# nrsyed/pytorch-yolov3

Hardware: AMD Instinct MI355X
Metric: frames/sec (608x608) (higher is better)
Workload: dtype bf16

## Files before the change

pytorch-yolov3_amd/csrc/conv_fused.hip:

```cpp
#include "common.h"
#include <type_traits>

namespace {

constexpr int kTO = 16;
constexpr int kSR = 2 * kTO + 1;
constexpr int kIR = kSR + 2;
constexpr int kInPitch = 144;
constexpr int kStemPitch = 80;
constexpr int kW1Pitch = 608;
constexpr int kNStem = kSR * kSR;
constexpr int kNFrag = (kNStem + 15) / 16;
constexpr int kThreads = 512;
constexpr int kInBytes = kIR * kInPitch * 2;
constexpr int kPatchElems = kIR * kIR * 3;
constexpr int kPre = (kPatchElems + kThreads - 1) / kThreads;
constexpr int kLds = 2 * kInBytes + kNStem * kStemPitch + 64 * kW1Pitch + 512;

template <typename T>
struct FusedArgs {
  const unsigned char *in;
  int H, W, batch;
  const T *w0;
  const float *sc0, *bi0;
  uint32_t flags0;
  const T *w1;
  int k_ld1;
  const float *sc1, *bi1;
  uint32_t flags1;
  T *out;
  int out_ld, Ho, Wo;
  int tiles_x, tiles_y, n_tiles;
  int dbg;
};

template <typename T>
__device__ __forceinline__ u32x2 bn_leaky_pack4(const f32x4 &a, const f32x4 &sc, const f32x4 &bi) {
  const f32x2 lo = f32x2{a[0], a[1]} * f32x2{sc[0], sc[1]} + f32x2{bi[0], bi[1]};
  const f32x2 hi = f32x2{a[2], a[3]} * f32x2{sc[2], sc[3]} + f32x2{bi[2], bi[3]};
  const f32x2 tl = lo * Y3_LEAKY_SLOPE, th = hi * Y3_LEAKY_SLOPE;
  return y3_pack4<T>(y3_vmax(lo[0], tl[0]), y3_vmax(lo[1], tl[1]), y3_vmax(hi[0], th[0]), y3_vmax(hi[1], th[1]));
}

template <typename T>
__global__ __launch_bounds__(kThreads) void conv_stem_s2_fused_kernel(FusedArgs<T> p) {
  typedef typename H16<T>::v8 V8;
  extern __shared__ __attribute__((aligned(16))) char smem[];
  T *in_tile = reinterpret_cast<T *>(smem);
  char *stem = smem + 2 * kInBytes;
  char *w1s = stem + kNStem * kStemPitch;
  T *lut = reinterpret_cast<T *>(w1s + 64 * kW1Pitch);

  const int tid = threadIdx.x, lane = tid & 63;
  const int wave = __builtin_amdgcn_readfirstlane(tid >> 6);
  const int fr = lane & 15, fq = lane >> 4;

  for (int i = tid; i < 64 * 36; i += kThreads) {
    const int co = i / 36, ch = i - co * 36;
    *reinterpret_cast<u32x4 *>(w1s + co * kW1Pitch + ch * 16) =
        *reinterpret_cast<const u32x4 *>(reinterpret_cast<const char *>(p.w1) + ((long long)co * p.k_ld1) * 2 + ch * 16);
  }
  V8 w0a[2], w0b[2];
#pragma unroll
  for (int st = 0; st < 2; ++st)
#pragma unroll
    for (int j = 0; j < 8; ++j) {
      const int k = st * 32 + fq * 8 + j;
      const int ky = k / 12, rem = k - ky * 12, kx = rem >> 2, c = rem & 3;
      const bool live = k < 36 && c < 3;
      const int kold = live ? ky * 9 + kx * 3 + c : 0;
      const T za = p.w0[(0 + fr) * 32 + kold], zb = p.w0[(16 + fr) * 32 + kold];
      w0a[st][j] = live ? za : (T)0.f;
      w0b[st][j] = live ? zb : (T)0.f;
    }
  int off_lo, off_hi;
  {
    const int k0 = fq * 8, k1 = fq * 8 + 4;
    off_lo = (k0 / 12) * kInPitch + (k0 % 12);
    off_hi = (k1 / 12) * kInPitch + (k1 % 12);
  }
  const int off_s1 = 2 * kInPitch + 8;
  const int cq = fq * 4;
  f32x4 sc0[2], bi0[2];
#pragma unroll
  for (int ni = 0; ni < 2; ++ni) {
    sc0[ni] = *reinterpret_cast<const f32x4 *>(p.sc0 + ni * 16 + cq);
    bi0[ni] = *reinterpret_cast<const f32x4 *>(p.bi0 + ni * 16 + cq);
  }

  int pr_row[kPre], pr_col[kPre], pr_dst[kPre];
  uint32_t pr_goff[kPre];
#pragma unroll
  for (int j = 0; j < kPre; ++j) {
    const int i = tid + j * kThreads;
    const int r = i / (kIR * 3), cb = i - r * (kIR * 3);
    pr_row[j] = r;
    pr_col[j] = cb;
    pr_goff[j] = (uint32_t)(r * p.W * 3 + cb);
    pr_dst[j] = r * kInPitch + (cb / 3) * 4 + (cb % 3);
  }
  const bool pr_last_live = tid + (kPre - 1) * kThreads < kPatchElems;
  auto tile_coords = [&](int tile, int &tx, int &ty, int &b) {
    int t = tile;
    tx = t % p.tiles_x;
    t /= p.tiles_x;
    ty = t % p.tiles_y;
    b = t / p.tiles_y;
  };
  auto patch_fetch = [&](int tile, unsigned char (&pre)[kPre]) {
    int tx, ty, b;
    tile_coords(tile, tx, ty, b);
    const int iy0 = 2 * ty * kTO - 2, ixb0 = (2 * tx * kTO - 2) * 3;
    const bool interior = iy0 >= 0 && iy0 + kIR <= p.H && ixb0 >= 0 && ixb0 + kIR * 3 <= p.W * 3;
    if (interior) {
      const unsigned char *base = p.in + ((long long)b * p.H + iy0) * p.W * 3 + ixb0;
#pragma unroll
      for (int j = 0; j < kPre; ++j) pre[j] = (j < kPre - 1 || pr_last_live) ? base[pr_goff[j]] : (unsigned char)0;
    } else {
#pragma unroll
      for (int j = 0; j < kPre; ++j) {
        const int iy = iy0 + pr_row[j], ixb = ixb0 + pr_col[j];
        unsigned char v = 0;
        if ((j < kPre - 1 || pr_last_live) && (unsigned)iy < (unsigned)p.H && ixb >= 0 && ixb < p.W * 3)
          v = p.in[((long long)b * p.H + iy) * p.W * 3 + ixb];
        pre[j] = v;
      }
    }
  };
  auto patch_store = [&](int buf, const unsigned char (&pre)[kPre]) {
    T *dst = in_tile + buf * (kIR * kInPitch);
#pragma unroll
    for (int j = 0; j < kPre; ++j)
      if (j < kPre - 1 || pr_last_live) dst[pr_dst[j]] = lut[pre[j]];
  };

  for (int i = tid; i < 2 * kIR * kInPitch / 2; i += kThreads) reinterpret_cast<uint32_t *>(in_tile)[i] = 0u;
  if (tid < 256) lut[tid] = (T)((float)tid / 255.0f);
  __syncthreads();
  int tile = blockIdx.x;
  int buf = 0;
  if (tile < p.n_tiles) {
    unsigned char pre[kPre];
    patch_fetch(tile, pre);
    patch_store(0, pre);
  }
  for (; tile < p.n_tiles; tile += gridDim.x) {
    int tx, ty, b;
    tile_coords(tile, tx, ty, b);
    const int oy0 = ty * kTO, ox0 = tx * kTO;
    __syncthreads();

    const T *patch = in_tile + buf * (kIR * kInPitch);
    const bool stem_inside = 2 * oy0 - 1 >= 0 && 2 * oy0 - 1 + kSR <= p.H && 2 * ox0 - 1 >= 0 && 2 * ox0 - 1 + kSR <= p.W;
    constexpr int kFG = 3;
    constexpr int kFragIters = (kNFrag + kThreads / 64 - 1) / (kThreads / 64);
    static_assert(kFragIters % kFG == 0, "fragment groups");
#pragma unroll 1
    for (int g = 0; g < ((p.dbg & 1) ? 0 : kFragIters); g += kFG) {
      u32x2 lo[kFG], hi[kFG], s1[kFG];
      int qv[kFG], syv[kFG], sxv[kFG];
#pragma unroll
      for (int j = 0; j < kFG; ++j) {
        const int q = (wave + (g + j) * (kThreads / 64)) * 16 + fr;
        const int qc = q < kNStem ? q : kNStem - 1;
        const int sy = qc / kSR, sx = qc - sy * kSR;
        const T *base = patch + sy * kInPitch + sx * 4;
        lo[j] = *reinterpret_cast<const u32x2 *>(base + off_lo);
        hi[j] = *reinterpret_cast<const u32x2 *>(base + off_hi);
        s1[j] = *reinterpret_cast<const u32x2 *>(base + off_s1);
        qv[j] = q;
        syv[j] = sy;
        sxv[j] = sx;
      }
      f32x4 acc0[kFG], acc1[kFG];
#pragma unroll
      for (int j = 0; j < kFG; ++j) {
        const V8 xf0 = __builtin_bit_cast(V8, u32x4{lo[j][0], lo[j][1], hi[j][0], hi[j][1]});
        acc0[j] = H16<T>::mfma(w0a[0], xf0, f32x4{0.f, 0.f, 0.f, 0.f});
        acc1[j] = H16<T>::mfma(w0b[0], xf0, f32x4{0.f, 0.f, 0.f, 0.f});
      }
#pragma unroll
      for (int j = 0; j < kFG; ++j) {
        const V8 xf1 = __builtin_bit_cast(V8, fq == 0 ? u32x4{s1[j][0], s1[j][1], 0u, 0u} : u32x4{0u, 0u, 0u, 0u});
        acc0[j] = H16<T>::mfma(w0a[1], xf1, acc0[j]);
        acc1[j] = H16<T>::mfma(w0b[1], xf1, acc1[j]);
      }
#pragma unroll
      for (int j = 0; j < kFG; ++j) {
        if (qv[j] < kNStem) {
          bool inside = true;
          if (!stem_inside) {
            const int gy = 2 * oy0 - 1 + syv[j], gx = 2 * ox0 - 1 + sxv[j];
            inside = (unsigned)gy < (unsigned)p.H && (unsigned)gx < (unsigned)p.W;
          }
#pragma unroll
          for (int ni = 0; ni < 2; ++ni) {
            u32x2 o = bn_leaky_pack4<T>(ni ? acc1[j] : acc0[j], sc0[ni], bi0[ni]);
            if (!inside) o = u32x2{0u, 0u};
            *reinterpret_cast<u32x2 *>(stem + qv[j] * kStemPitch + (ni * 16 + cq) * 2) = o;
          }
        }
      }
    }
    const int next_tile = tile + gridDim.x;
    unsigned char pre[kPre];
    if (next_tile < p.n_tiles && !(p.dbg & 8)) patch_fetch(next_tile, pre);
    __syncthreads();

    f32x4 acc[2][4];
#pragma unroll
    for (int mi = 0; mi < 2; ++mi)
#pragma unroll
      for (int nf = 0; nf < 4; ++nf) acc[mi][nf] = f32x4{0.f, 0.f, 0.f, 0.f};
#pragma unroll
    for (int tap = 0; tap < ((p.dbg & 2) ? 0 : 9); ++tap) {
      const int ky = tap / 3, kx = tap - ky * 3;
      u32x4 xf[2], wf[4];
#pragma unroll
      for (int mi = 0; mi < 2; ++mi) {
        const int q = (2 * (2 * wave + mi) + ky) * kSR + 2 * fr + kx;
        xf[mi] = *reinterpret_cast<const u32x4 *>(stem + q * kStemPitch + fq * 16);
      }
#pragma unroll
      for (int nf = 0; nf < 4; ++nf)
        wf[nf] = *reinterpret_cast<const u32x4 *>(w1s + (nf * 16 + fr) * kW1Pitch + tap * 64 + fq * 16);
#pragma unroll
      for (int mi = 0; mi < 2; ++mi)
#pragma unroll
        for (int nf = 0; nf < 4; ++nf)
          acc[mi][nf] = H16<T>::mfma(__builtin_bit_cast(V8, wf[nf]),
                                                                __builtin_bit_cast(V8, xf[mi]), acc[mi][nf]);
    }
    if (next_tile < p.n_tiles) patch_store(buf ^ 1, pre);
    __syncthreads();

#pragma unroll
    for (int nf = 0; nf < 4; ++nf) {
      const f32x4 s1 = *reinterpret_cast<const f32x4 *>(p.sc1 + nf * 16 + cq);
      const f32x4 b1 = *reinterpret_cast<const f32x4 *>(p.bi1 + nf * 16 + cq);
#pragma unroll
      for (int mi = 0; mi < 2; ++mi) {
        const int px = (2 * wave + mi) * kTO + fr;
        const int co = nf * 16 + cq;
        *reinterpret_cast<u32x2 *>(stem + px * 128 + (((co >> 3) ^ (px & 7)) << 4) + (co & 7) * 2) =
            bn_leaky_pack4<T>(acc[mi][nf], s1, b1);
      }
    }
    __syncthreads();
#pragma unroll
    for (int j = 0; j < kTO * kTO * 8 / kThreads; ++j) {
      const int i = tid + j * kThreads;
      const int px = i >> 3, ch = i & 7;
      const int oy = oy0 + (px >> 4), ox = ox0 + (px & 15);
      if (oy < p.Ho && ox < p.Wo && !(p.dbg & 4)) {
        const u32x4 v = *reinterpret_cast<const u32x4 *>(stem + px * 128 + ((ch ^ (px & 7)) << 4));
        *reinterpret_cast<u32x4 *>(p.out + (((long long)b * p.Ho + oy) * p.Wo + ox) * p.out_ld + ch * 8) = v;
      }
    }
    buf ^= 1;
  }
}


constexpr int kPX = 16, kPY = 8;
constexpr int kPSX = 2 * kPX + 1;
constexpr int kPSY = 2 * kPY + 1;
constexpr int kPIX = kPSX + 2, kPIY = kPSY + 2;
constexpr int kPNStem = kPSX * kPSY;
constexpr int kPNFrag = (kPNStem + 15) / 16;
constexpr int kPInBytes = kPIY * kInPitch * 2;
constexpr int kPStemBytes = kPNStem * kStemPitch;
constexpr int kPStage = 8 * 16 * 128;
constexpr int kPLds = 2 * kPInBytes + 2 * kPStemBytes + 64 * kW1Pitch + 512 + kPStage;
static_assert(kPLds <= 160 * 1024, "LDS budget");
static_assert(kPX == 16 && kPY == 8, "one 16-pixel output row per conv wave");

template <typename T, int NC>
__global__ __launch_bounds__(1024) void conv_stem_s2_ws_kernel(FusedArgs<T> p) {
  typedef typename H16<T>::v8 V8;
  constexpr int NS = 16 - NC, NT = 1024;
  constexpr int MR = kPY / NC;
  constexpr int kIters = (kPNFrag + NS - 1) / NS;
  constexpr int kPairs = kPIY * ((kPIX * 3 + 1) / 2);
  constexpr int kPre = (kPairs + 64 * NS - 1) / (64 * NS);
  extern __shared__ __attribute__((aligned(16))) char smem[];
  char *in_tile = smem;
  char *stem0 = smem + 2 * kPInBytes;
  char *w1s = stem0 + 2 * kPStemBytes;
  T *lut = reinterpret_cast<T *>(w1s + 64 * kW1Pitch);
  char *stage = reinterpret_cast<char *>(lut) + 512;

  const int tid = threadIdx.x, lane = tid & 63;
  const int wave = __builtin_amdgcn_readfirstlane(tid >> 6);
  const int fr = lane & 15, fq = lane >> 4;
  const bool is_stem = wave >= NC;

  for (int i = tid; i < 64 * 36; i += NT) {
    const int j = i / 36, ch = i - j * 36;
    const int co = y3_pair_perm(j);
    *reinterpret_cast<u32x4 *>(w1s + j * kW1Pitch + ch * 16) =
        *reinterpret_cast<const u32x4 *>(reinterpret_cast<const char *>(p.w1) + ((long long)co * p.k_ld1) * 2 + ch * 16);
  }
  for (int i = tid; i < 2 * kPInBytes / 4; i += NT) reinterpret_cast<uint32_t *>(in_tile)[i] = 0u;
  if (tid < 256) lut[tid] = (T)((float)tid / 255.0f);
  __syncthreads();
  const int tile0 = blockIdx.x, stride = gridDim.x;
  if (tile0 >= p.n_tiles) return;
  struct TilePos { int tile, tx, ty, b; };
  auto pos_of = [&](int tile) {
    TilePos t;
    t.tile = tile;
    t.tx = tile % p.tiles_x;
    const int r = tile / p.tiles_x;
    t.ty = r % p.tiles_y;
    t.b = r / p.tiles_y;
    return t;
  };
  const TilePos dpos = pos_of(stride);
  auto advance = [&](TilePos &t) {
    t.tile += stride;
    t.tx += dpos.tx;
    int c = t.tx >= p.tiles_x ? 1 : 0;
    t.tx -= c ? p.tiles_x : 0;
    t.ty += dpos.ty + c;
    c = t.ty >= p.tiles_y ? 1 : 0;
    t.ty -= c ? p.tiles_y : 0;
    t.b += dpos.b + c;
  };

  if (is_stem) {
    const int sw = wave - NC, stid = tid - 64 * NC;
    V8 w0a[2], w0b[2];
#pragma unroll
    for (int st = 0; st < 2; ++st)
#pragma unroll
      for (int j = 0; j < 8; ++j) {
        const int k = st * 32 + fq * 8 + j;
        const int ky = k / 12, rem = k - ky * 12, kx = rem >> 2, c = rem & 3;
        const bool live = k < 36 && c < 3;
        const int kold = live ? ky * 9 + kx * 3 + c : 0;
        const T za = p.w0[y3_pair_perm(fr) * 32 + kold], zb = p.w0[y3_pair_perm(16 + fr) * 32 + kold];
        w0a[st][j] = live ? za : (T)0.f;
        w0b[st][j] = live ? zb : (T)0.f;
      }
    int off_lo, off_hi;
    {
      const int k0 = fq * 8, k1 = fq * 8 + 4;
      off_lo = ((k0 / 12) * kInPitch + (k0 % 12)) * 2;
      off_hi = ((k1 / 12) * kInPitch + (k1 % 12)) * 2;
    }
    constexpr int off_s1 = (2 * kInPitch + 8) * 2;
    f32x4 sc0[2], bi0[2];
#pragma unroll
    for (int ni = 0; ni < 2; ++ni) {
      sc0[ni] = *reinterpret_cast<const f32x4 *>(p.sc0 + fq * 8 + ni * 4);
      bi0[ni] = *reinterpret_cast<const f32x4 *>(p.bi0 + fq * 8 + ni * 4);
    }
    int fr_patch[kIters];
    uint32_t fr_live = 0;
#pragma unroll
    for (int j = 0; j < kIters; ++j) {
      const int q = (sw + NS * j) * 16 + fr;
      const int qc = q < kPNStem ? q : kPNStem - 1;
      const int sy = qc / kPSX, sx = qc - sy * kPSX;
      fr_patch[j] = (sy * kInPitch + sx * 4) * 2;
      fr_live |= (q < kPNStem ? 1u : 0u) << j;
    }
    int stem_wr = ((sw * 16 + fr) * kStemPitch) + fq * 16;
    asm volatile("" : "+v"(stem_wr));
    constexpr int kRowPairs = (kPIX * 3 + 1) / 2;
    int pr_dst[kPre];
    uint32_t pr_goff[kPre];
    uint32_t pr_one = 0;
#pragma unroll
    for (int j = 0; j < kPre; ++j) {
      const int i = stid + j * 64 * NS;
      const int r = i / kRowPairs, cb = 2 * (i - r * kRowPairs);
      pr_goff[j] = (uint32_t)(r * p.W * 3 + cb);
      pr_dst[j] = (r * kInPitch + (cb / 3) * 4 + (cb % 3)) * 2 | (cb % 3 == 2 ? 1 : 0);
      pr_one |= (cb + 1 >= kPIX * 3 ? 1u : 0u) << j;
    }
    const bool pr_last_live = stid + (kPre - 1) * 64 * NS < kPairs;
    const bool pairs_aligned = ((p.W * 3) & 1) == 0 && (reinterpret_cast<size_t>(p.in) & 1) == 0;
    auto patch_fetch = [&](const TilePos &t, unsigned short (&pre)[kPre]) {
      const int tx = t.tx, ty = t.ty, b = t.b;
      const int iy0 = 2 * ty * kPY - 2, ixb0 = (2 * tx * kPX - 2) * 3;
      const bool interior = pairs_aligned && iy0 >= 0 && iy0 + kPIY <= p.H && ixb0 >= 0 && ixb0 + 2 * kRowPairs <= p.W * 3;
      if (interior) {
        const unsigned char *base = p.in + ((long long)b * p.H + iy0) * p.W * 3 + ixb0;
#pragma unroll
        for (int j = 0; j < kPre; ++j)
          pre[j] = (j < kPre - 1 || pr_last_live) ? *reinterpret_cast<const unsigned short *>(base + pr_goff[j]) : (unsigned short)0;
      } else {
#pragma unroll
        for (int j = 0; j < kPre; ++j) {
          const int i = stid + j * 64 * NS;
          const int r = i / kRowPairs, cb = 2 * (i - r * kRowPairs);
          const int iy = iy0 + r, ixb = ixb0 + cb;
          unsigned int v = 0;
          if ((j < kPre - 1 || pr_last_live) && (unsigned)iy < (unsigned)p.H) {
            const unsigned char *row = p.in + ((long long)b * p.H + iy) * p.W * 3;
            if (ixb >= 0 && ixb < p.W * 3) v = row[ixb];
            if (ixb + 1 >= 0 && ixb + 1 < p.W * 3 && cb + 1 < kPIX * 3) v |= (unsigned int)row[ixb + 1] << 8;
          }
          pre[j] = (unsigned short)v;
        }
      }
    };
    auto patch_store = [&](int buf, const unsigned short (&pre)[kPre]) {
      char *dst = in_tile + buf * kPInBytes;
#pragma unroll
      for (int j = 0; j < kPre; ++j)
        if (j < kPre - 1 || pr_last_live) {
          char *d = dst + (pr_dst[j] & ~1);
          *reinterpret_cast<T *>(d) = lut[pre[j] & 255];
          if (!((pr_one >> j) & 1u)) *reinterpret_cast<T *>(d + 2 + 2 * (pr_dst[j] & 1)) = lut[pre[j] >> 8];
        }
    };
    auto stem_image = [&](const char *patch, char *img, const TilePos &t) {
      const int oy0 = t.ty * kPY, ox0 = t.tx * kPX;
      const bool all_inside = 2 * oy0 - 1 >= 0 && 2 * oy0 - 1 + kPSY <= p.H && 2 * ox0 - 1 >= 0 && 2 * ox0 - 1 + kPSX <= p.W;
      auto group = [&](auto g0, auto cnt) {
        constexpr int g = decltype(g0)::value, G = decltype(cnt)::value;
        u32x2 lo[G], hi[G], s1[G];
#pragma unroll
        for (int j = 0; j < G; ++j) {
          const char *base = patch + fr_patch[g + j];
          lo[j] = *reinterpret_cast<const u32x2 *>(base + off_lo);
          hi[j] = *reinterpret_cast<const u32x2 *>(base + off_hi);
          s1[j] = *reinterpret_cast<const u32x2 *>(base + off_s1);
        }
        f32x4 a0[G], a1[G];
#pragma unroll
        for (int j = 0; j < G; ++j) {
          const V8 xf0 = __builtin_bit_cast(V8, u32x4{lo[j][0], lo[j][1], hi[j][0], hi[j][1]});
          a0[j] = H16<T>::mfma(w0a[0], xf0, f32x4{0.f, 0.f, 0.f, 0.f});
          a1[j] = H16<T>::mfma(w0b[0], xf0, f32x4{0.f, 0.f, 0.f, 0.f});
        }
#pragma unroll
        for (int j = 0; j < G; ++j) {
          const V8 xf1 = __builtin_bit_cast(V8, u32x4{s1[j][0], s1[j][1], s1[j][0], s1[j][1]});
          a0[j] = H16<T>::mfma(w0a[1], xf1, a0[j]);
          a1[j] = H16<T>::mfma(w0b[1], xf1, a1[j]);
        }
#pragma unroll
        for (int j = 0; j < G; ++j) {
          u32x2 o0 = bn_leaky_pack4<T>(a0[j], sc0[0], bi0[0]);
          u32x2 o1 = bn_leaky_pack4<T>(a1[j], sc0[1], bi0[1]);
          if (!all_inside) {
            const int q = (sw + NS * (g + j)) * 16 + fr;
            const int qc = q < kPNStem ? q : kPNStem - 1;
            const int sy = qc / kPSX, sx = qc - sy * kPSX;
            const int gy = 2 * oy0 - 1 + sy, gx = 2 * ox0 - 1 + sx;
            if (!((unsigned)gy < (unsigned)p.H && (unsigned)gx < (unsigned)p.W)) {
              o0 = u32x2{0u, 0u};
              o1 = u32x2{0u, 0u};
            }
          }
          if ((fr_live >> (g + j)) & 1u) {
            char *dst = img + stem_wr + (g + j) * (NS * 16 * kStemPitch);
            *reinterpret_cast<u32x4 *>(dst) = u32x4{o0[0], o0[1], o1[0], o1[1]};
          }
        }
      };
      using std::integral_constant;
      static_assert(kIters == 5 || kIters == 3, "fragment groups");
      group(integral_constant<int, 0>{}, integral_constant<int, 3>{});
      if constexpr (kIters == 5) group(integral_constant<int, 3>{}, integral_constant<int, 2>{});
    };

    unsigned short pre[4][kPre];
    TilePos fpos = pos_of(tile0);
    TilePos ipos = fpos;
    {
      patch_fetch(fpos, pre[0]);
      patch_store(0, pre[0]);
      advance(fpos);
      if (fpos.tile < p.n_tiles) {
        patch_fetch(fpos, pre[1]);
        patch_store(1, pre[1]);
      }
      advance(fpos);
    }
    __builtin_amdgcn_s_waitcnt(0xC07F);
    __builtin_amdgcn_s_barrier();
#pragma unroll
    for (int k = 0; k < 3; ++k) {
      if (fpos.tile < p.n_tiles) patch_fetch(fpos, pre[k]);
      advance(fpos);
    }
    stem_image(in_tile, stem0, ipos);
    advance(ipos);
    __builtin_amdgcn_s_waitcnt(0xC07F);
    __builtin_amdgcn_s_barrier();
    int par = 0;
    Y3_STAMP_DECL
    auto step = [&](auto setc) {
      constexpr int set = decltype(setc)::value;
      if (fpos.tile < p.n_tiles) patch_fetch(fpos, pre[(set + 3) & 3]);
      advance(fpos);
      Y3_STAMP(0);
      const bool more = ipos.tile < p.n_tiles;
      if (more) stem_image(in_tile + (par ^ 1) * kPInBytes, stem0 + (par ^ 1) * kPStemBytes, ipos);
      advance(ipos);
      __builtin_amdgcn_s_waitcnt(0xC07F);
      Y3_STAMP(1);
      if (ipos.tile < p.n_tiles) patch_store(par, pre[set]);
      __builtin_amdgcn_s_waitcnt(0xC07F);
      Y3_STAMP(2);
      __builtin_amdgcn_s_barrier();
      Y3_STAMP(3);
      par ^= 1;
      return more;
    };
    using std::integral_constant;
    for (;;) {
      if (!step(integral_constant<int, 0>{})) break;
      if (!step(integral_constant<int, 1>{})) break;
      if (!step(integral_constant<int, 2>{})) break;
      if (!step(integral_constant<int, 3>{})) break;
    }
#ifdef Y3_STAMPS
    if (tid == 64 * NC) for (int _i = 0; _i < 4; ++_i) atomicAdd(&g_y3_stamps[_i], _st_acc[_i]);
#endif
    return;
  }

  const int a_rd = ((2 * wave * MR) * kPSX + 2 * fr) * kStemPitch + fq * 16;
  const int b_rd = fr * kW1Pitch + fq * 16;
  char *my_stage = stage + wave * (MR * 16 * 128);
  f32x4 s1v[4], b1v[4];
#pragma unroll
  for (int nf = 0; nf < 4; ++nf) {
    s1v[nf] = *reinterpret_cast<const f32x4 *>(p.sc1 + (nf >> 1) * 32 + fq * 8 + (nf & 1) * 4);
    b1v[nf] = *reinterpret_cast<const f32x4 *>(p.bi1 + (nf >> 1) * 32 + fq * 8 + (nf & 1) * 4);
  }
  __builtin_amdgcn_s_waitcnt(0xC07F);
  __builtin_amdgcn_s_barrier();
  __builtin_amdgcn_s_barrier();
  uint32_t st_off[2];
#pragma unroll
  for (int k = 0; k < 2; ++k) st_off[k] = (uint32_t)((((lane >> 3) + 8 * k) * p.out_ld + (lane & 7) * 8) * 2);
  int par = 0;
  Y3_STAMP_DECL
  for (TilePos pos = pos_of(tile0); pos.tile < p.n_tiles; advance(pos)) {
    const int b = pos.b;
    const int oy0 = pos.ty * kPY, ox0 = pos.tx * kPX;
    const char *img = stem0 + par * kPStemBytes;
    f32x4 acc[MR][4];
#pragma unroll
    for (int mr = 0; mr < MR; ++mr)
#pragma unroll
      for (int nf = 0; nf < 4; ++nf) acc[mr][nf] = f32x4{0.f, 0.f, 0.f, 0.f};
#pragma unroll
    for (int tap = 0; tap < 9; ++tap) {
      const int ky = tap / 3, kx = tap - ky * 3;
      u32x4 xf[MR], wf[4];
#pragma unroll
      for (int mr = 0; mr < MR; ++mr)
        xf[mr] = *reinterpret_cast<const u32x4 *>(img + a_rd + ((2 * mr + ky) * kPSX + kx) * kStemPitch);
#pragma unroll
      for (int nf = 0; nf < 4; ++nf)
        wf[nf] = *reinterpret_cast<const u32x4 *>(w1s + b_rd + nf * 16 * kW1Pitch + tap * 64);
#pragma unroll
      for (int mr = 0; mr < MR; ++mr)
#pragma unroll
        for (int nf = 0; nf < 4; ++nf)
          acc[mr][nf] = H16<T>::mfma(__builtin_bit_cast(V8, wf[nf]),
                                                                __builtin_bit_cast(V8, xf[mr]), acc[mr][nf]);
    }
    Y3_STAMP(4);
#pragma unroll
    for (int mr = 0; mr < MR; ++mr)
#pragma unroll
      for (int k = 0; k < 2; ++k) {
        const u32x2 lo = bn_leaky_pack4<T>(acc[mr][2 * k], s1v[2 * k], b1v[2 * k]);
        const u32x2 hi = bn_leaky_pack4<T>(acc[mr][2 * k + 1], s1v[2 * k + 1], b1v[2 * k + 1]);
        *reinterpret_cast<u32x4 *>(my_stage + mr * 2048 + fr * 128 + (((k * 4 + fq) ^ (fr & 7)) << 4)) = u32x4{lo[0], lo[1], hi[0], hi[1]};
      }
    __builtin_amdgcn_wave_barrier();
#pragma unroll
    for (int mr = 0; mr < MR; ++mr) {
      const int oy = oy0 + wave * MR + mr;
      char *row = reinterpret_cast<char *>(p.out + (((long long)b * p.Ho + oy) * p.Wo + ox0) * p.out_ld);
      const bool full = ox0 + kPX <= p.Wo;
#pragma unroll
      for (int k = 0; k < 2; ++k) {
        const int px = (lane >> 3) + 8 * k, ch = lane & 7;
        const u32x4 v = *reinterpret_cast<const u32x4 *>(my_stage + mr * 2048 + px * 128 + ((ch ^ (px & 7)) << 4));
        if (oy < p.Ho && (full || ox0 + px < p.Wo)) *reinterpret_cast<u32x4 *>(row + st_off[k]) = v;
      }
    }
    __builtin_amdgcn_wave_barrier();
    __builtin_amdgcn_s_waitcnt(0xC07F);
    Y3_STAMP(5);
    __builtin_amdgcn_s_barrier();
    Y3_STAMP(6);
    par ^= 1;
  }
#ifdef Y3_STAMPS
  if (tid == 0) {
    for (int _i = 4; _i < 7; ++_i) atomicAdd(&g_y3_stamps[_i], _st_acc[_i]);
    atomicAdd(&g_y3_stamps[7], 1ull);
  }
#endif
}

constexpr int kRT = 16;
constexpr int kRP = kRT + 2;
constexpr int kRNP = kRP * kRP;
constexpr int kRFrag = (kRNP + 15) / 16;
constexpr int kYPitch = 96;
constexpr int kXBytes = kRNP * 128;
constexpr int kYBytes = 32768;
constexpr int kRLds = kXBytes + kYBytes + 64 * kW1Pitch;
constexpr int kXPre = (kRNP * 8 + kThreads - 1) / kThreads;
static_assert(kRNP * kYPitch <= kYBytes && kRT * kRT * 128 <= kYBytes, "image / staging tile must fit");

template <typename T>
struct ResArgs {
  const T *x;
  int H, W, batch, x_ld;
  const T *w2; int k_ld2; const float *sc2, *bi2;
  const T *w3; int k_ld3; const float *sc3, *bi3;
  T *out;
  int out_ld;
  int tiles_x, tiles_y, n_tiles;
};

template <typename T>
__global__ __launch_bounds__(kThreads) void conv_resblock_fused_kernel(ResArgs<T> p) {
  typedef typename H16<T>::v8 V8;
  extern __shared__ __attribute__((aligned(16))) char smem[];
  char *xt = smem;
  char *yt = smem + kXBytes;
  char *w3s = yt + kYBytes;

  const int tid = threadIdx.x, lane = tid & 63;
  const int wave = __builtin_amdgcn_readfirstlane(tid >> 6);
  const int fr = lane & 15, fq = lane >> 4;

  for (int i = tid; i < 64 * 36; i += kThreads) {
    const int j = i / 36, ch = i - j * 36;
    const int co = y3_pair_perm(j);
    *reinterpret_cast<u32x4 *>(w3s + j * kW1Pitch + ch * 16) =
        *reinterpret_cast<const u32x4 *>(reinterpret_cast<const char *>(p.w3) + ((long long)co * p.k_ld3) * 2 + ch * 16);
  }
  u32x4 w2f[2][2];
#pragma unroll
  for (int ni = 0; ni < 2; ++ni)
#pragma unroll
    for (int ks = 0; ks < 2; ++ks)
      w2f[ni][ks] = *reinterpret_cast<const u32x4 *>(reinterpret_cast<const char *>(p.w2) +
                                                    ((long long)y3_pair_perm(ni * 16 + fr) * p.k_ld2 + ks * 32 + fq * 8) * 2);
  f32x4 sc2[2], bi2[2];
#pragma unroll
  for (int ni = 0; ni < 2; ++ni) {
    sc2[ni] = *reinterpret_cast<const f32x4 *>(p.sc2 + fq * 8 + ni * 4);
    bi2[ni] = *reinterpret_cast<const f32x4 *>(p.bi2 + fq * 8 + ni * 4);
  }

  auto tile_origin = [&](int tile, int &b, int &oy0, int &ox0) {
    const int tx = tile % p.tiles_x;
    tile /= p.tiles_x;
    oy0 = (tile % p.tiles_y) * kRT;
    b = tile / p.tiles_y;
    ox0 = tx * kRT;
  };
  int xrc[kXPre];
  uint32_t xoff[kXPre];
  int xlds[kXPre];
#pragma unroll
  for (int j = 0; j < kXPre; ++j) {
    const int i = tid + j * kThreads;
    const int px = i >> 3, c = i & 7;
    const int r = px / kRP, cc = px - r * kRP;
    xrc[j] = i < kRNP * 8 ? (r << 8) | cc : -1;
    xoff[j] = ((uint32_t)(r * p.W + cc) * (uint32_t)p.x_ld) * 2u + (uint32_t)c * 16u;
    xlds[j] = px * 128 + ((c ^ (px & 7)) << 4);
  }
  constexpr int kAFr = (kRFrag + kThreads / 64 - 1) / (kThreads / 64);
  int a_rd[kAFr], a_rc[kAFr], a_wr[kAFr];
#pragma unroll
  for (int fs = 0; fs < kAFr; ++fs) {
    const int q = (wave + fs * (kThreads / 64)) * 16 + fr;
    const int qc = q < kRNP ? q : kRNP - 1;
    const int r = qc / kRP, cc = qc - r * kRP;
    a_rd[fs] = qc * 128 + ((fq ^ (qc & 7)) << 4);
    a_rc[fs] = (r << 8) | cc;
    a_wr[fs] = q < kRNP ? q * kYPitch + fq * 16 : -1;
  }
  constexpr int kOutPer = kRT * kRT * 8 / kThreads;
  int opx[kOutPer], olds[kOutPer];
  uint32_t ooff[kOutPer];
#pragma unroll
  for (int j = 0; j < kOutPer; ++j) {
    const int i = tid + j * kThreads;
    const int px = i >> 3, ch = i & 7;
    opx[j] = px;
    ooff[j] = ((uint32_t)((px >> 4) * p.W + (px & 15)) * (uint32_t)p.out_ld + (uint32_t)ch * 8u) * 2u;
    olds[j] = px * 128 + ((ch ^ (px & 7)) << 4);
  }
  auto x_fetch = [&](int tile, u32x4 (&pre)[kXPre]) {
    int b, oy0, ox0;
    tile_origin(tile, b, oy0, ox0);
    const char *base = reinterpret_cast<const char *>(p.x) + ((((long long)b * p.H + (oy0 - 1)) * p.W + (ox0 - 1)) * p.x_ld) * 2;
#pragma unroll
    for (int j = 0; j < kXPre; ++j) {
      const int gy = oy0 - 1 + (xrc[j] >> 8), gx = ox0 - 1 + (xrc[j] & 255);
      u32x4 v = {0u, 0u, 0u, 0u};
      if (xrc[j] >= 0 && (unsigned)gy < (unsigned)p.H && (unsigned)gx < (unsigned)p.W)
        v = *reinterpret_cast<const u32x4 *>(base + xoff[j]);
      pre[j] = v;
    }
  };
  auto x_store = [&](const u32x4 (&pre)[kXPre]) {
#pragma unroll
    for (int j = 0; j < kXPre; ++j)
      if (xrc[j] >= 0) *reinterpret_cast<u32x4 *>(xt + xlds[j]) = pre[j];
  };

  int tile = blockIdx.x;
  if (tile < p.n_tiles) {
    u32x4 pre[kXPre];
    x_fetch(tile, pre);
    x_store(pre);
  }
  for (; tile < p.n_tiles; tile += gridDim.x) {
    int b, oy0, ox0;
    tile_origin(tile, b, oy0, ox0);
    __syncthreads();

#pragma unroll
    for (int fs = 0; fs < kAFr; ++fs) {
      if (wave + fs * (kThreads / 64) >= kRFrag) break;
      const u32x4 xa = *reinterpret_cast<const u32x4 *>(xt + a_rd[fs]);
      const u32x4 xb = *reinterpret_cast<const u32x4 *>(xt + (a_rd[fs] ^ 64));
      const bool inside = (unsigned)(oy0 - 1 + (a_rc[fs] >> 8)) < (unsigned)p.H && (unsigned)(ox0 - 1 + (a_rc[fs] & 255)) < (unsigned)p.W;
      u32x2 o[2];
#pragma unroll
      for (int ni = 0; ni < 2; ++ni) {
        f32x4 a = {0.f, 0.f, 0.f, 0.f};
        a = H16<T>::mfma(__builtin_bit_cast(V8, w2f[ni][0]), __builtin_bit_cast(V8, xa), a);
        a = H16<T>::mfma(__builtin_bit_cast(V8, w2f[ni][1]), __builtin_bit_cast(V8, xb), a);
        o[ni] = bn_leaky_pack4<T>(a, sc2[ni], bi2[ni]);
        if (!inside) o[ni] = u32x2{0u, 0u};
      }
      if (a_wr[fs] >= 0) *reinterpret_cast<u32x4 *>(yt + a_wr[fs]) = u32x4{o[0][0], o[0][1], o[1][0], o[1][1]};
    }
    const int next_tile = tile + gridDim.x;
    u32x4 pre[kXPre];
    if (next_tile < p.n_tiles) x_fetch(next_tile, pre);
    __syncthreads();

    f32x4 acc[2][4];
#pragma unroll
    for (int mi = 0; mi < 2; ++mi)
#pragma unroll
      for (int nf = 0; nf < 4; ++nf) acc[mi][nf] = f32x4{0.f, 0.f, 0.f, 0.f};
#pragma unroll
    for (int tap = 0; tap < 9; ++tap) {
      const int ky = tap / 3, kx = tap - ky * 3;
      u32x4 xf[2], wf[4];
#pragma unroll
      for (int mi = 0; mi < 2; ++mi) {
        const int q = (2 * wave + mi + ky) * kRP + fr + kx;
        xf[mi] = *reinterpret_cast<const u32x4 *>(yt + q * kYPitch + fq * 16);
      }
#pragma unroll
      for (int nf = 0; nf < 4; ++nf)
        wf[nf] = *reinterpret_cast<const u32x4 *>(w3s + (nf * 16 + fr) * kW1Pitch + tap * 64 + fq * 16);
#pragma unroll
      for (int mi = 0; mi < 2; ++mi)
#pragma unroll
        for (int nf = 0; nf < 4; ++nf)
          acc[mi][nf] = H16<T>::mfma(__builtin_bit_cast(V8, wf[nf]),
                                                                __builtin_bit_cast(V8, xf[mi]), acc[mi][nf]);
    }
    __syncthreads();

#pragma unroll
    for (int k = 0; k < 2; ++k) {
      f32x4 s3[2], b3[2];
#pragma unroll
      for (int h = 0; h < 2; ++h) {
        s3[h] = *reinterpret_cast<const f32x4 *>(p.sc3 + k * 32 + fq * 8 + h * 4);
        b3[h] = *reinterpret_cast<const f32x4 *>(p.bi3 + k * 32 + fq * 8 + h * 4);
      }
#pragma unroll
      for (int mi = 0; mi < 2; ++mi) {
        const int oyl = 2 * wave + mi;
        const int pp = (oyl + 1) * kRP + fr + 1;
        const u32x4 xr = *reinterpret_cast<const u32x4 *>(xt + pp * 128 + (((k * 4 + fq) ^ (pp & 7)) << 4));
        float v[8];
        y3_bn_act8(v, acc[mi][2 * k], acc[mi][2 * k + 1], s3[0], s3[1], b3[0], b3[1], Y3_ACT_LEAKY);
        y3_add8<T>(v, xr);
        const int px = oyl * kRT + fr;
        *reinterpret_cast<u32x4 *>(yt + px * 128 + (((k * 4 + fq) ^ (px & 7)) << 4)) = y3_pack8<T>(v);
      }
    }
    __syncthreads();
    {
      char *obase = reinterpret_cast<char *>(p.out) + ((((long long)b * p.H + oy0) * p.W + ox0) * p.out_ld) * 2;
#pragma unroll
      for (int j = 0; j < kOutPer; ++j) {
        const int oy = oy0 + (opx[j] >> 4), ox = ox0 + (opx[j] & 15);
        if (oy < p.H && ox < p.W) *reinterpret_cast<u32x4 *>(obase + ooff[j]) = *reinterpret_cast<const u32x4 *>(yt + olds[j]);
      }
    }
    if (next_tile < p.n_tiles) x_store(pre);
  }
}

}


static int launch_stem_s2(const y3_op *ops, const y3_step &st, const void *d_in, const void *, hipStream_t s);
static int launch_resblock(const y3_op *ops, const y3_step &st, const void *, const void *, hipStream_t s);

struct FusedGeom { int tiles_x, tiles_y, n_tiles; long long grid; };
static FusedGeom fused_geom(int out_w, int out_h, int batch, int tw, int th) {
  FusedGeom g;
  g.tiles_x = y3_ceil_div(out_w, tw);
  g.tiles_y = y3_ceil_div(out_h, th);
  g.n_tiles = g.tiles_x * g.tiles_y * batch;
  const int n_cu = y3_device_cus();
  g.grid = g.n_tiles < n_cu ? g.n_tiles : n_cu;
  return g;
}
static FusedGeom stem_s2_geom(const y3_op &op1, bool pipelined) {
  return fused_geom(op1.out_w, op1.out_h, op1.batch, pipelined ? kPX : kTO, pipelined ? kPY : kTO);
}
static FusedGeom resblock_geom(const y3_op &op0) { return fused_geom(op0.in_w, op0.in_h, op0.batch, kRT, kRT); }

bool y3_choose_conv_fused_stem_s2(const y3_op &op0, const y3_op &op1, const y3_options &o, y3_step &st) {
  if (!o.fuse_stem) return false;
  if (!y3_conv_stem_mfma_supported(op0) || op0.out_c != 32 || (op0.flags & Y3_F_RESIDUAL)) return false;
  if (!(op0.flags & Y3_F_LEAKY) || !(op1.flags & Y3_F_LEAKY)) return false;
  if ((op0.flags | op1.flags) & (Y3_F_MISH | Y3_F_LOGISTIC)) return false;
  if (op1.kind != Y3_OP_CONV || op1.dtype != op0.dtype || op1.ksize != 3 || op1.stride != 2 || op1.pad != 1) return false;
  if (op1.in_c != 32 || op1.out_c != 64 || op1.out_ld % 8 != 0 || op1.out_ld < 64) return false;
  if (op1.flags & (Y3_F_RESIDUAL | Y3_F_OUT_F32 | Y3_F_IN_NCHW_F32 | Y3_F_IN_NHWC_U8BGR | Y3_F_PLAN_INPUT)) return false;
  if (op1.d_in != op0.d_out || op1.in_h != op0.out_h || op1.in_w != op0.out_w || op1.batch != op0.batch) return false;
  if (op1.k_ld < 288 || op1.cout_pad < 64) return false;
  if (op1.out_h != (op1.in_h + 2 - 3) / 2 + 1 || op1.out_w != (op1.in_w + 2 - 3) / 2 + 1) return false;
  if ((long long)kIR * op0.in_w * 3 >= (1ll << 31) || op1.out_ld >= (1 << 24)) return false;
  st.launch = launch_stem_s2;
  st.name = op0.dtype == Y3_F16 ? "conv_stem_s2_fused_u8_f16" : "conv_stem_s2_fused_u8_bf16";
  st.pipelined = o.fuse_stem != 2;
  st.dims = {stem_s2_geom(op1, st.pipelined).grid, st.pipelined ? 1024 : kThreads, (size_t)(st.pipelined ? kPLds : kLds)};
  return true;
}

static int launch_stem_s2(const y3_op *ops, const y3_step &st, const void *d_in, const void *, hipStream_t s) {
  const y3_op &op0 = ops[0], &op1 = ops[1];
  return y3_by_dtype16(op0.dtype, [&](auto tag) {
    typedef decltype(tag) T;
    FusedArgs<T> a;
    a.in = static_cast<const unsigned char *>(d_in);
    a.H = op0.in_h; a.W = op0.in_w; a.batch = op0.batch;
    a.w0 = static_cast<const T *>(op0.d_weight);
    a.sc0 = op0.d_scale; a.bi0 = op0.d_bias; a.flags0 = op0.flags;
    a.w1 = static_cast<const T *>(op1.d_weight);
    a.k_ld1 = op1.k_ld;
    a.sc1 = op1.d_scale; a.bi1 = op1.d_bias; a.flags1 = op1.flags;
    a.out = static_cast<T *>(op1.d_out);
    a.out_ld = op1.out_ld; a.Ho = op1.out_h; a.Wo = op1.out_w;
    a.dbg = 0;
    const FusedGeom g = stem_s2_geom(op1, st.pipelined);
    a.tiles_x = g.tiles_x; a.tiles_y = g.tiles_y; a.n_tiles = g.n_tiles;
    if (!st.pipelined) return y3_launch<conv_stem_s2_fused_kernel<T>>(st.dims, s, a);
    return y3_launch<conv_stem_s2_ws_kernel<T, 4>>(st.dims, s, a);
  });
}

bool y3_choose_conv_fused_resblock(const y3_op &op0, const y3_op &op1, const y3_options &o, y3_step &st) {
  if (!o.fuse_stem) return false;
  if (op0.kind != Y3_OP_CONV || op1.kind != Y3_OP_CONV || !y3_is16(op0.dtype) || op1.dtype != op0.dtype) return false;
  if (op0.ksize != 1 || op0.stride != 1 || op0.in_c != 64 || op0.out_c != 32) return false;
  if (op1.ksize != 3 || op1.stride != 1 || op1.pad != 1 || op1.in_c != 32 || op1.out_c != 64) return false;
  const uint32_t bad = Y3_F_OUT_F32 | Y3_F_IN_NCHW_F32 | Y3_F_IN_NHWC_U8BGR | Y3_F_PLAN_INPUT;
  if ((op0.flags & (bad | Y3_F_RESIDUAL)) || (op1.flags & bad)) return false;
  if (!(op0.flags & Y3_F_LEAKY) || !(op1.flags & Y3_F_LEAKY) || !(op1.flags & Y3_F_RESIDUAL)) return false;
  if ((op0.flags | op1.flags) & (Y3_F_MISH | Y3_F_LOGISTIC)) return false;
  if (op1.d_in != op0.d_out || op1.d_res != op0.d_in || op1.res_ld != op0.in_ld) return false;
  if (op0.in_h != op1.in_h || op0.in_w != op1.in_w || op0.batch != op1.batch) return false;
  if (op0.out_h != op0.in_h || op0.out_w != op0.in_w || op1.out_h != op1.in_h || op1.out_w != op1.in_w) return false;
  if (op0.in_ld % 8 != 0 || op1.out_ld % 8 != 0 || op0.in_ld < 64 || op1.out_ld < 64) return false;
  if (op0.k_ld < 64 || op1.k_ld < 288 || op0.cout_pad < 32 || op1.cout_pad < 64) return false;
  if ((long long)(kRT + 2) * op0.in_w * (op0.in_ld > op1.out_ld ? op0.in_ld : op1.out_ld) * 2 >= (1ll << 32)) return false;
  st.launch = launch_resblock;
  st.dims = {resblock_geom(op0).grid, kThreads, kRLds};
  st.name = Y3_KNAME(op0.dtype, "conv_resblock_fused_", "_64_32_64");
  return true;
}

static int launch_resblock(const y3_op *ops, const y3_step &st, const void *, const void *, hipStream_t s) {
  const y3_op &op0 = ops[0], &op1 = ops[1];
  return y3_by_dtype16(op0.dtype, [&](auto tag) {
    typedef decltype(tag) T;
    ResArgs<T> a;
    a.x = static_cast<const T *>(op0.d_in);
    a.H = op0.in_h; a.W = op0.in_w; a.batch = op0.batch; a.x_ld = op0.in_ld;
    a.w2 = static_cast<const T *>(op0.d_weight); a.k_ld2 = op0.k_ld; a.sc2 = op0.d_scale; a.bi2 = op0.d_bias;
    a.w3 = static_cast<const T *>(op1.d_weight); a.k_ld3 = op1.k_ld; a.sc3 = op1.d_scale; a.bi3 = op1.d_bias;
    a.out = static_cast<T *>(op1.d_out);
    a.out_ld = op1.out_ld;
    const FusedGeom g = resblock_geom(op0);
    a.tiles_x = g.tiles_x; a.tiles_y = g.tiles_y; a.n_tiles = g.n_tiles;
    return y3_launch<conv_resblock_fused_kernel<T>>(st.dims, s, a);
  });
}

Y3_STAMP_READER(y3_debug_stamps_fused)
```

Measured before the change: 5730.

## Keep 3x3 weights in registers and restructure resblock kernel schedule

The fused residual-block kernel now holds the 3x3 conv weights in per-wave registers, splitting waves into row and output-channel halves, instead of reading them from LDS on every tap. The output is staged in a separate LDS region, so the next tile's patch store can happen before the global write-out, which removes one barrier. Tile positions are advanced incrementally instead of with div/mod. Interior tiles skip bounds checks, loads are made unconditional using a safe address, and the BN constants come from LDS. The price is much higher register pressure from 18 weight fragments per thread, which could lower occupancy or cause spills.

```diff
diff --git a/pytorch-yolov3_amd/csrc/conv_fused.hip b/pytorch-yolov3_amd/csrc/conv_fused.hip
--- a/pytorch-yolov3_amd/csrc/conv_fused.hip
+++ b/pytorch-yolov3_amd/csrc/conv_fused.hip
@@ -613,9 +613,10 @@
 constexpr int kYPitch = 96;
 constexpr int kXBytes = kRNP * 128;
 constexpr int kYBytes = 32768;
-constexpr int kRLds = kXBytes + kYBytes + 64 * kW1Pitch;
+constexpr int kRStage = 64 * kW1Pitch;
+constexpr int kRLds = kXBytes + kYBytes + kRStage;
 constexpr int kXPre = (kRNP * 8 + kThreads - 1) / kThreads;
-static_assert(kRNP * kYPitch <= kYBytes && kRT * kRT * 128 <= kYBytes, "image / staging tile must fit");
+static_assert(kRNP * kYPitch <= kYBytes && kRT * kRT * 128 + 512 <= kRStage, "image / staging tile and the 3x3's constants must fit");
 
 template <typename T>
 struct ResArgs {
@@ -634,18 +635,22 @@
   extern __shared__ __attribute__((aligned(16))) char smem[];
   char *xt = smem;
   char *yt = smem + kXBytes;
-  char *w3s = yt + kYBytes;
+  char *stage = yt + kYBytes;
+  float *cst = reinterpret_cast<float *>(stage + kRT * kRT * 128);
 
   const int tid = threadIdx.x, lane = tid & 63;
   const int wave = __builtin_amdgcn_readfirstlane(tid >> 6);
   const int fr = lane & 15, fq = lane >> 4;
-
-  for (int i = tid; i < 64 * 36; i += kThreads) {
-    const int j = i / 36, ch = i - j * 36;
-    const int co = y3_pair_perm(j);
-    *reinterpret_cast<u32x4 *>(w3s + j * kW1Pitch + ch * 16) =
-        *reinterpret_cast<const u32x4 *>(reinterpret_cast<const char *>(p.w3) + ((long long)co * p.k_ld3) * 2 + ch * 16);
-  }
+  const int wr = wave >> 1, wk = wave & 1;
+
+  u32x4 w3f[9][2];
+#pragma unroll
+  for (int tap = 0; tap < 9; ++tap)
+#pragma unroll
+    for (int h = 0; h < 2; ++h)
+      w3f[tap][h] = *reinterpret_cast<const u32x4 *>(reinterpret_cast<const char *>(p.w3) +
+                                                     ((long long)y3_pair_perm((2 * wk + h) * 16 + fr) * p.k_ld3 + tap * 32 + fq * 8) * 2);
+  if (tid < 128) cst[tid] = tid < 64 ? p.sc3[tid] : p.bi3[tid - 64];
   u32x4 w2f[2][2];
 #pragma unroll
   for (int ni = 0; ni < 2; ++ni)
@@ -660,16 +665,31 @@
     bi2[ni] = *reinterpret_cast<const f32x4 *>(p.bi2 + fq * 8 + ni * 4);
   }
 
-  auto tile_origin = [&](int tile, int &b, int &oy0, int &ox0) {
-    const int tx = tile % p.tiles_x;
-    tile /= p.tiles_x;
-    oy0 = (tile % p.tiles_y) * kRT;
-    b = tile / p.tiles_y;
-    ox0 = tx * kRT;
+  struct TilePos { int tile, tx, ty, b; };
+  auto pos_of = [&](int tile) {
+    TilePos t;
+    t.tile = tile;
+    t.tx = tile % p.tiles_x;
+    const int r = tile / p.tiles_x;
+    t.ty = r % p.tiles_y;
+    t.b = r / p.tiles_y;
+    return t;
+  };
+  const TilePos dpos = pos_of(gridDim.x);
+  auto advance = [&](TilePos &t) {
+    t.tile += gridDim.x;
+    t.tx += dpos.tx;
+    int c = t.tx >= p.tiles_x ? 1 : 0;
+    t.tx -= c ? p.tiles_x : 0;
+    t.ty += dpos.ty + c;
+    c = t.ty >= p.tiles_y ? 1 : 0;
+    t.ty -= c ? p.tiles_y : 0;
+    t.b += dpos.b + c;
   };
   int xrc[kXPre];
   uint32_t xoff[kXPre];
-  int xlds[kXPre];
+  const int xlds = (tid >> 3) * 128 + (((tid & 7) ^ ((tid >> 3) & 7)) << 4);
+  const uint32_t xsafe = ((uint32_t)(p.W + 1) * (uint32_t)p.x_ld) * 2u + (uint32_t)(tid & 7) * 16u;
 #pragma unroll
   for (int j = 0; j < kXPre; ++j) {
     const int i = tid + j * kThreads;
@@ -677,65 +697,71 @@
     const int r = px / kRP, cc = px - r * kRP;
     xrc[j] = i < kRNP * 8 ? (r << 8) | cc : -1;
     xoff[j] = ((uint32_t)(r * p.W + cc) * (uint32_t)p.x_ld) * 2u + (uint32_t)c * 16u;
-    xlds[j] = px * 128 + ((c ^ (px & 7)) << 4);
   }
   constexpr int kAFr = (kRFrag + kThreads / 64 - 1) / (kThreads / 64);
-  int a_rd[kAFr], a_rc[kAFr], a_wr[kAFr];
+  const int a_rd = (wave * 16 + fr) * 128 + ((fq ^ (fr & 7)) << 4);
+  const int a_wr = (wave * 16 + fr) * kYPitch + fq * 16;
+  int a_rc[kAFr];
 #pragma unroll
   for (int fs = 0; fs < kAFr; ++fs) {
     const int q = (wave + fs * (kThreads / 64)) * 16 + fr;
     const int qc = q < kRNP ? q : kRNP - 1;
     const int r = qc / kRP, cc = qc - r * kRP;
-    a_rd[fs] = qc * 128 + ((fq ^ (qc & 7)) << 4);
     a_rc[fs] = (r << 8) | cc;
-    a_wr[fs] = q < kRNP ? q * kYPitch + fq * 16 : -1;
-  }
+  }
+  static_assert((kAFr * (kThreads / 64) * 16 - 1) * 128 + 128 <= kXBytes + kYBytes, "phase A reads stay inside the patch and image regions");
+  const int b_rd = (4 * wr * kRP + fr) * kYPitch + fq * 16;
   constexpr int kOutPer = kRT * kRT * 8 / kThreads;
-  int opx[kOutPer], olds[kOutPer];
-  uint32_t ooff[kOutPer];
-#pragma unroll
-  for (int j = 0; j < kOutPer; ++j) {
-    const int i = tid + j * kThreads;
-    const int px = i >> 3, ch = i & 7;
-    opx[j] = px;
-    ooff[j] = ((uint32_t)((px >> 4) * p.W + (px & 15)) * (uint32_t)p.out_ld + (uint32_t)ch * 8u) * 2u;
-    olds[j] = px * 128 + ((ch ^ (px & 7)) << 4);
-  }
-  auto x_fetch = [&](int tile, u32x4 (&pre)[kXPre]) {
-    int b, oy0, ox0;
-    tile_origin(tile, b, oy0, ox0);
-    const char *base = reinterpret_cast<const char *>(p.x) + ((((long long)b * p.H + (oy0 - 1)) * p.W + (ox0 - 1)) * p.x_ld) * 2;
+  const int orow = tid >> 7, ocol = (tid >> 3) & 15;
+  const uint32_t ooff = ((uint32_t)(orow * p.W + ocol) * (uint32_t)p.out_ld + (uint32_t)(tid & 7) * 8u) * 2u;
+  const uint32_t ostep = (uint32_t)(4 * p.W) * (uint32_t)p.out_ld * 2u;
+  const int olds = (tid >> 3) * 128 + (((tid & 7) ^ ((tid >> 3) & 7)) << 4);
+  auto whole_patch = [&](const TilePos &t) {
+    return t.ty > 0 && t.tx > 0 && t.ty * kRT + kRT + 1 <= p.H && t.tx * kRT + kRT + 1 <= p.W;
+  };
+  auto x_fetch = [&](const TilePos &t, u32x4 (&pre)[kXPre]) {
+    const int oy0 = t.ty * kRT, ox0 = t.tx * kRT;
+    const char *base = reinterpret_cast<const char *>(p.x) + ((((long long)t.b * p.H + (oy0 - 1)) * p.W + (ox0 - 1)) * p.x_ld) * 2;
+    const bool whole = whole_patch(t);
+    int keep = 0;
 #pragma unroll
     for (int j = 0; j < kXPre; ++j) {
       const int gy = oy0 - 1 + (xrc[j] >> 8), gx = ox0 - 1 + (xrc[j] & 255);
-      u32x4 v = {0u, 0u, 0u, 0u};
-      if (xrc[j] >= 0 && (unsigned)gy < (unsigned)p.H && (unsigned)gx < (unsigned)p.W)
-        v = *reinterpret_cast<const u32x4 *>(base + xoff[j]);
-      pre[j] = v;
-    }
+      const bool ok = ((j + 1) * kThreads <= kRNP * 8 || xrc[j] >= 0) && (whole || ((unsigned)gy < (unsigned)p.H && (unsigned)gx < (unsigned)p.W));
+      keep |= ok ? 1 << j : 0;
+      uint32_t off = ok ? xoff[j] : xsafe;
+      asm volatile("" : "+v"(off));
+      pre[j] = *reinterpret_cast<const u32x4 *>(base + off);
+    }
+    return keep;
   };
-  auto x_store = [&](const u32x4 (&pre)[kXPre]) {
+  auto x_store = [&](u32x4 (&pre)[kXPre], int keep, bool whole) {
+    if (!whole) {
+#pragma unroll
+      for (int j = 0; j < kXPre; ++j)
+        if (!(keep & (1 << j))) pre[j] = u32x4{0u, 0u, 0u, 0u};
+    }
 #pragma unroll
     for (int j = 0; j < kXPre; ++j)
-      if (xrc[j] >= 0) *reinterpret_cast<u32x4 *>(xt + xlds[j]) = pre[j];
+      if ((j + 1) * kThreads <= kRNP * 8 || xrc[j] >= 0) *reinterpret_cast<u32x4 *>(xt + xlds + j * 8192) = pre[j];
   };
 
-  int tile = blockIdx.x;
-  if (tile < p.n_tiles) {
+  TilePos pos = pos_of(blockIdx.x);
+  if (pos.tile < p.n_tiles) {
     u32x4 pre[kXPre];
-    x_fetch(tile, pre);
-    x_store(pre);
-  }
-  for (; tile < p.n_tiles; tile += gridDim.x) {
-    int b, oy0, ox0;
-    tile_origin(tile, b, oy0, ox0);
+    const int keep = x_fetch(pos, pre);
+    x_store(pre, keep, whole_patch(pos));
+  }
+  Y3_STAMP_DECL
+  while (pos.tile < p.n_tiles) {
+    const int b = pos.b, oy0 = pos.ty * kRT, ox0 = pos.tx * kRT;
     __syncthreads();
+    Y3_STAMP(0);
 
 #pragma unroll
     for (int fs = 0; fs < kAFr; ++fs) {
-      if (wave + fs * (kThreads / 64) >= kRFrag) break;
-      const u32x4 xa = *reinterpret_cast<const u32x4 *>(xt + a_rd[fs]);
-      const u32x4 xb = *reinterpret_cast<const u32x4 *>(xt + (a_rd[fs] ^ 64));
+      const u32x4 xa = *reinterpret_cast<const u32x4 *>(xt + a_rd + fs * 16384);
+      const u32x4 xb = *reinterpret_cast<const u32x4 *>(xt + (a_rd ^ 64) + fs * 16384);
       const bool inside = (unsigned)(oy0 - 1 + (a_rc[fs] >> 8)) < (unsigned)p.H && (unsigned)(ox0 - 1 + (a_rc[fs] & 255)) < (unsigned)p.W;
       u32x2 o[2];
 #pragma unroll
@@ -746,70 +772,71 @@
         o[ni] = bn_leaky_pack4<T>(a, sc2[ni], bi2[ni]);
         if (!inside) o[ni] = u32x2{0u, 0u};
       }
-      if (a_wr[fs] >= 0) *reinterpret_cast<u32x4 *>(yt + a_wr[fs]) = u32x4{o[0][0], o[0][1], o[1][0], o[1][1]};
-    }
-    const int next_tile = tile + gridDim.x;
+      if ((wave + fs * (kThreads / 64)) * 16 + fr < kRNP)
+        *reinterpret_cast<u32x4 *>(yt + a_wr + fs * 12288) = u32x4{o[0][0], o[0][1], o[1][0], o[1][1]};
+    }
+    TilePos next = pos;
+    advance(next);
+    const TilePos fetch = next.tile < p.n_tiles ? next : pos;
     u32x4 pre[kXPre];
-    if (next_tile < p.n_tiles) x_fetch(next_tile, pre);
+    const int keep = x_fetch(fetch, pre);
+    Y3_STAMP(1);
     __syncthreads();
-
-    f32x4 acc[2][4];
-#pragma unroll
-    for (int mi = 0; mi < 2; ++mi)
-#pragma unroll
-      for (int nf = 0; nf < 4; ++nf) acc[mi][nf] = f32x4{0.f, 0.f, 0.f, 0.f};
+    Y3_STAMP(2);
+
+    f32x4 acc[4][2];
+#pragma unroll
+    for (int mi = 0; mi < 4; ++mi)
+#pragma unroll
+      for (int h = 0; h < 2; ++h) acc[mi][h] = f32x4{0.f, 0.f, 0.f, 0.f};
 #pragma unroll
     for (int tap = 0; tap < 9; ++tap) {
       const int ky = tap / 3, kx = tap - ky * 3;
-      u32x4 xf[2], wf[4];
-#pragma unroll
-      for (int mi = 0; mi < 2; ++mi) {
-        const int q = (2 * wave + mi + ky) * kRP + fr + kx;
-        xf[mi] = *reinterpret_cast<const u32x4 *>(yt + q * kYPitch + fq * 16);
-      }
-#pragma unroll
-      for (int nf = 0; nf < 4; ++nf)
-        wf[nf] = *reinterpret_cast<const u32x4 *>(w3s + (nf * 16 + fr) * kW1Pitch + tap * 64 + fq * 16);
-#pragma unroll
-      for (int mi = 0; mi < 2; ++mi)
-#pragma unroll
-        for (int nf = 0; nf < 4; ++nf)
-          acc[mi][nf] = H16<T>::mfma(__builtin_bit_cast(V8, wf[nf]),
-                                                                __builtin_bit_cast(V8, xf[mi]), acc[mi][nf]);
-    }
+      u32x4 xf[4];
+#pragma unroll
+      for (int mi = 0; mi < 4; ++mi)
+        xf[mi] = *reinterpret_cast<const u32x4 *>(yt + b_rd + ((mi + ky) * kRP + kx) * kYPitch);
+#pragma unroll
+      for (int mi = 0; mi < 4; ++mi)
+#pragma unroll
+        for (int h = 0; h < 2; ++h)
+          acc[mi][h] = H16<T>::mfma(__builtin_bit_cast(V8, w3f[tap][h]), __builtin_bit_cast(V8, xf[mi]), acc[mi][h]);
+    }
+    Y3_STAMP(3);
+
+    f32x4 sc3[2], bi3[2];
+#pragma unroll
+    for (int h = 0; h < 2; ++h) {
+      sc3[h] = *reinterpret_cast<const f32x4 *>(cst + wk * 32 + fq * 8 + h * 4);
+      bi3[h] = *reinterpret_cast<const f32x4 *>(cst + 64 + wk * 32 + fq * 8 + h * 4);
+    }
+#pragma unroll
+    for (int mi = 0; mi < 4; ++mi) {
+      const int oyl = 4 * wr + mi;
+      const int pp = (oyl + 1) * kRP + fr + 1;
+      const u32x4 xr = *reinterpret_cast<const u32x4 *>(xt + pp * 128 + (((wk * 4 + fq) ^ (pp & 7)) << 4));
+      float v[8];
+      y3_bn_act8(v, acc[mi][0], acc[mi][1], sc3[0], sc3[1], bi3[0], bi3[1], Y3_ACT_LEAKY);
+      y3_add8<T>(v, xr);
+      const int px = oyl * kRT + fr;
+      *reinterpret_cast<u32x4 *>(stage + px * 128 + (((wk * 4 + fq) ^ (px & 7)) << 4)) = y3_pack8<T>(v);
+    }
+    Y3_STAMP(4);
     __syncthreads();
-
-#pragma unroll
-    for (int k = 0; k < 2; ++k) {
-      f32x4 s3[2], b3[2];
-#pragma unroll
-      for (int h = 0; h < 2; ++h) {
-        s3[h] = *reinterpret_cast<const f32x4 *>(p.sc3 + k * 32 + fq * 8 + h * 4);
-        b3[h] = *reinterpret_cast<const f32x4 *>(p.bi3 + k * 32 + fq * 8 + h * 4);
-      }
-#pragma unroll
-      for (int mi = 0; mi < 2; ++mi) {
-        const int oyl = 2 * wave + mi;
-        const int pp = (oyl + 1) * kRP + fr + 1;
-        const u32x4 xr = *reinterpret_cast<const u32x4 *>(xt + pp * 128 + (((k * 4 + fq) ^ (pp & 7)) << 4));
-        float v[8];
-        y3_bn_act8(v, acc[mi][2 * k], acc[mi][2 * k + 1], s3[0], s3[1], b3[0], b3[1], Y3_ACT_LEAKY);
-        y3_add8<T>(v, xr);
-        const int px = oyl * kRT + fr;
-        *reinterpret_cast<u32x4 *>(yt + px * 128 + (((k * 4 + fq) ^ (px & 7)) << 4)) = y3_pack8<T>(v);
-      }
-    }
-    __syncthreads();
+    x_store(pre, keep, whole_patch(fetch));
+    Y3_STAMP(5);
     {
       char *obase = reinterpret_cast<char *>(p.out) + ((((long long)b * p.H + oy0) * p.W + ox0) * p.out_ld) * 2;
-#pragma unroll
-      for (int j = 0; j < kOutPer; ++j) {
-        const int oy = oy0 + (opx[j] >> 4), ox = ox0 + (opx[j] & 15);
-        if (oy < p.H && ox < p.W) *reinterpret_cast<u32x4 *>(obase + ooff[j]) = *reinterpret_cast<const u32x4 *>(yt + olds[j]);
-      }
-    }
-    if (next_tile < p.n_tiles) x_store(pre);
-  }
+      const bool col_in = ox0 + ocol < p.W;
+#pragma unroll
+      for (int j = 0; j < kOutPer; ++j)
+        if (oy0 + orow + 4 * j < p.H && col_in)
+          *reinterpret_cast<u32x4 *>(obase + ooff + j * ostep) = *reinterpret_cast<const u32x4 *>(stage + olds + j * 8192);
+    }
+    Y3_STAMP(6);
+    pos = next;
+  }
+  Y3_STAMP_COUNT();
 }
 
 }
```

After: 5785 (median of 5 runs). Within noise of the previous version (+1.0%).
